# thnak/image_super_resolution

Hardware: AMD Instinct MI355X
Metric: 4x SR megapixels/sec (HR output) + PSNR vs reference CPU path (higher is better)
Workload: dtype fp16; 1 GPU; ResNet(16, 0.2, scaleRate=4) RRDB inference, 128x128->512x512; global_batch=16, per_gpu_batch=16, lr_size=128, scale=4, parallelism=dp1 (independent tile shards), streams_per_gpu=1, hip_graph=True, trunk=persistent chain kernel, storage=fp16 activations and packed weights, fp32 accumulation

## Files before the change

### image_super_resolution_amd/csrc/trunk.hip

```cpp
#include "trunk_common.h"

namespace isr {

size_t trunk_state_words(int n, int ha, int wa) {
    const size_t tiles = (size_t)n * (ha / tk::TH) * (wa / tk::TW);
    return trunk_rec_off((int)tiles) + 1024 * 16;
}

__global__ __launch_bounds__(1024) void trunk_prep_kernel(const isr_conv_desc* layers, const int32_t* kinds, int nl,
                                                          int n, int ha, int wa, unsigned* state, int th,
                                                          int h16) {
    extern __shared__ __attribute__((aligned(16))) char smem[];
    unsigned* err = reinterpret_cast<unsigned*>(smem);
    const int L = threadIdx.x;
    const int nbx = wa / tk::TW, nby = ha / th, ntiles = n * nbx * nby;
    const size_t ro = trunk_rec_off(ntiles);
    if (L == 0) *err = 0;
    __syncthreads();
    const isr_conv_desc& g0 = layers[0];
    if (L < nl) {
        const isr_conv_desc& d = layers[L];
        unsigned e = 0;
        auto same_geo = [&](const isr_view& v) {
            return v.hp == g0.x.hp && v.wp == g0.x.wp && v.cs == g0.x.cs && v.pad == g0.x.pad && v.coff % 16 == 0 &&
                   v.pad >= 1;
        };
        const int kind = kinds[L];
        const bool masked = kind == 2;
        if (d.n != n || d.ha != ha || d.wa != wa || d.h != g0.h || d.w != g0.w) e |= 1;
        if (!same_geo(d.x) || !same_geo(d.y) || (d.r2.data && !same_geo(d.r2)) || (masked && !same_geo(d.m))) e |= 2;
        if (kind == 0 || kind == 2 ? d.cout != 32 : (kind == 1 ? d.cout != 64 : true)) e |= 4;
        if (d.cin % 16 || d.cin < 64 || d.cin / 16 > 120 || !d.bias || ((uintptr_t)d.bias & 15)) e |= 8;
        if (d.f16 != h16 || d.shuffle != 1 || d.x_sub2 || d.taps || d.y2.data || (d.m.data != nullptr) != masked ||
            (masked && (d.m_c0 != 0 || d.slope != 1.f || d.r1.data || d.r2.data || d.s1 != 1.f || d.s2 != 1.f)))
            e |= 16;
        int fold = 0;
        uint16_t idv = 0;
        if (d.r1.data) {
            const float inv = 1.f / d.s1;
            float back;
            if (h16) {
                const _Float16 hi = (_Float16)inv;
                idv = __builtin_bit_cast(uint16_t, hi);
                back = (float)hi;
            } else {
                const __bf16 bi = (__bf16)inv;
                idv = __builtin_bit_cast(uint16_t, bi);
                back = (float)bi;
            }
            const bool alias = d.r1.data == d.x.data && d.r1.coff == d.x.coff && d.r1_cn == 0;
            if (!alias || kind != 1 || d.slope != 1.f || back != inv) e |= 32;
            fold = 1;
        } else if (d.r2.data) {
            e |= 32;
        }
        int first_new = tk::NEED_NONE;
        if (L > 0) {
            const isr_conv_desc& p = layers[L - 1];
            const int lo = p.y.coff, hi = p.y.coff + p.cout;
            first_new = d.cin / 16;
            if (p.y.data == d.x.data) {
                for (int c = 0; c < d.cin / 16; ++c) {
                    const int c0 = d.x.coff + 16 * c;
                    if (c0 < hi && lo < c0 + 16) {
                        first_new = c;
                        break;
                    }
                }
            }
        }
        TrunkRec rec;
        rec.x = (uint64_t)(uintptr_t)d.x.data;
        rec.y = (uint64_t)(uintptr_t)d.y.data;
        rec.w = (uint64_t)(uintptr_t)d.wpack;
        rec.b = (uint64_t)(uintptr_t)d.bias;
        rec.r2 = (uint64_t)(uintptr_t)(masked ? d.m.data : d.r2.data);
        rec.planes = (uint32_t)(d.x.coff / 16) | (uint32_t)(d.y.coff / 16) << 16;
        rec.shape = (uint32_t)((masked ? d.m.coff : d.r2.coff) / 16) | (uint32_t)(d.cin / 16) << 16 |
                    (uint32_t)(kind & 255) << 24;
        int form = EPI_GENERAL;
        if (kind == 0 && !d.r1.data && !d.r2.data && d.s2 == 1.f && d.slope > 0.f && d.slope < 1.f)
            form = EPI_GROWTH;
        else if (kind == 1 && fold && d.slope == 1.f)
            form = d.r2.data ? EPI_FINAL_R2 : (d.s2 == 1.f ? EPI_FINAL : EPI_FINAL_S2);
        rec.deps = (uint32_t)first_new | (uint32_t)fold << 8 | (uint32_t)form << 9 | (uint32_t)idv << 16;
        rec.slope = masked ? d.mslope : d.slope;
        rec.s1 = d.s1;
        rec.s2 = d.s2;
        const uint32_t* src = reinterpret_cast<const uint32_t*>(&rec);
        uint32_t* dst = state + ro + (size_t)L * 16;
#pragma unroll
        for (int i = 0; i < 16; ++i) dst[i] = src[i];
        if (e) atomicOr(err, e);
    }
    __syncthreads();
    if (L == 0) {
        const size_t plane = (size_t)g0.x.hp * g0.x.wp * 32;
        const unsigned e = *err | (plane >= 0x7fffffffull ? 64u : 0u) | (nl > 1024 ? 128u : 0u);
        uint32_t* geo = state + ro - 16;
        const int32_t gv[16] = {n, g0.h, g0.w, ha, wa, g0.x.hp, g0.x.wp, g0.x.cs / 16, g0.x.pad, nbx, nby, ntiles,
                                (int32_t)e, 0, 0, 0};
#pragma unroll
        for (int i = 0; i < 16; ++i) geo[i] = (uint32_t)gv[i];
        state[0] = state[0] + 1u;
    }
}

int trunk_prep_launch(const isr_chain_desc* cd, int th, hipStream_t s) {
    hipLaunchKernelGGL(trunk_prep_kernel, dim3(1), dim3(1024), 16, s, cd->layers, cd->kinds, cd->nl, cd->n, cd->ha,
                       cd->wa, cd->state, th, cd->f16 ? 1 : 0);
    return hipGetLastError() == hipSuccess ? 0 : -1;
}

#ifdef ISR_TUNING
__device__ unsigned long long* g_trunk_stamps;
#endif
__device__ __forceinline__ void trunk_stamp(int L, int t, int ntiles, int slot) {
#ifdef ISR_TUNING
    unsigned long long* p = g_trunk_stamps;
    if (p != nullptr && threadIdx.x == 0 && L >= 75 && L < 90) {
        unsigned long long v;
        asm volatile("s_memrealtime %0\n\ts_waitcnt lgkmcnt(0)" : "=s"(v)::"memory");
        p[((size_t)(L - 75) * ntiles + t) * 8 + slot] = v;
    }
#else
    (void)L, (void)t, (void)ntiles, (void)slot;
#endif
}

#ifdef ISR_TUNING
__device__ int g_trunk_knobs[4];
static int g_trunk_per_cu = 0;
__device__ __forceinline__ int trunk_abl_load() { return __builtin_amdgcn_readfirstlane(g_trunk_knobs[0]); }
#else
__device__ __forceinline__ int trunk_abl_load() { return 0; }
#endif

#ifdef ISR_TUNING
__device__ unsigned long long* g_item_stamps;
#endif
__device__ __forceinline__ void item_stamp(int L, int first_tile, int ch, int slot, int wm) {
#ifdef ISR_TUNING
    unsigned long long* p = g_item_stamps;
    const int w = wave_id();
    if (p != nullptr && first_tile && (threadIdx.x & 63) == 0 && (w == 0 || w == wm / 2) && (L == 77 || L == 79)) {
        const unsigned long long v = __builtin_amdgcn_s_memtime();
        p[((((size_t)blockIdx.x * 2 + (L == 79)) * 16 + ch) * 2 + (w != 0)) * 8 + slot] = v;
    }
#else
    (void)L, (void)first_tile, (void)ch, (void)slot, (void)wm;
#endif
}

struct TrunkArgs {
    unsigned* state;
    int rec_off;
    int nl;
    int acquire;
};


__device__ __forceinline__ void glds4(const void* gsrc, void* lds) {
    __builtin_amdgcn_global_load_lds(gsrc, ISR_LDS_PTR(lds), 4, 0, 0);
}

struct TK {
    static constexpr int WM = 4, R = 4, NST = 2;
    static constexpr int HALO_AUX = 16, STORE_AUX = 16;
    static constexpr int NT = 64 * WM;
    static constexpr int TH = tk::TH;
    static constexpr int HQ = (TH + 2) * tk::HC;
    static constexpr int HP = (HQ + 31) / 32;
    static_assert(R * WM == TH, "the waves cover the tile rows");
    static constexpr int HPW = (HP + WM - 1) / WM;
    static constexpr int WPW = (tk::WPF + WM - 1) / WM;
    static constexpr int SLOT = (HP + tk::WPF) * 1024;
    static constexpr int BIAS_OFF = NST * SLOT;
    static constexpr int LDS = BIAS_OFF + 4 * 256;
    static constexpr int BPC = 2;
    static_assert(BPC * LDS <= 163840, "LDS budget");
    static constexpr int WPS = BPC * WM / 4;
};

struct Src {
    const char* x;
    uint32_t h0;
    const char* w;
    const float* b;
    int wpc;
    uint32_t xbytes, wbytes;
};

struct TrunkCtx {
    unsigned* state;
    unsigned gen;
    int acquire;
    int hp, wp, cs16, pad, h, w, nbx, nby, ntiles;
    uint32_t pstride;
    uint32_t hoff[TK::HPW];
    int abl;
};

__device__ __forceinline__ Src src_of(const TrunkCtx& c, const_rec& rec, int t) {
    const int bx = t % c.nbx, tmp = t / c.nbx, by = tmp % c.nby, img = tmp / c.nby;
    Src s;
    s.x = (const char*)(uintptr_t)rec.x + (size_t)((uint32_t)img * c.cs16 + rec_xp(rec)) * c.pstride;
    s.h0 = (uint32_t)(((by * TK::TH - 1 + c.pad) * c.wp + (bx * tk::TW - 1 + c.pad)) * 32);
    s.w = (const char*)(uintptr_t)rec.w;
    s.b = (const float*)(uintptr_t)rec.b;
    s.wpc = rec_kind(rec) == 1 ? tk::WPF : tk::WPG;
    s.xbytes = c.pstride;
    s.wbytes = (uint32_t)(rec_nch(rec) * s.wpc * 1024);
    return s;
}

__device__ __forceinline__ uint32_t stage_pieces(const uint32_t* hoff, uint32_t pstride, int abl, const Src& s,
                                                 int chunk, int slot, bool with_bias, int bslot) {
    extern __shared__ __attribute__((aligned(16))) char smem[];
    const int wave = wave_id(), lane = threadIdx.x & 63;
    char* dst = smem + slot * TK::SLOT;
    uint32_t n = 0;
    const auto rx = rsrc_n(s.x + (size_t)chunk * pstride, s.xbytes);
    const uint32_t so = s.h0;
    if (!(abl & 1)) {
#pragma unroll
        for (int k = 0; k < TK::HPW; ++k) {
            const int j = wave + TK::WM * k;
            if (j < TK::HP) {
                __builtin_amdgcn_raw_ptr_buffer_load_lds(rx, ISR_LDS_PTR(dst + j * 1024), 16, hoff[k], so, 0, TK::HALO_AUX);
                ++n;
            }
        }
    }
    const auto rw = rsrc_n(s.w, s.wbytes);
    const uint32_t wo = (uint32_t)(chunk * s.wpc * 1024);
    char* wd = dst + TK::HP * 1024;
#pragma unroll
    for (int k = 0; k < TK::WPW; ++k) {
        const int j = wave + TK::WM * k;
        if (j < s.wpc && !(abl & 8)) {
            __builtin_amdgcn_raw_ptr_buffer_load_lds(rw, ISR_LDS_PTR(wd + j * 1024), 16, lane * 16, wo + j * 1024, 0, 0);
            ++n;
        }
    }
    if (with_bias && wave == 0) {
        if (lane < (s.wpc == tk::WPG ? 32 : 64))
            __builtin_amdgcn_raw_ptr_buffer_load_lds(rsrc_n(s.b, s.wpc == tk::WPG ? 128u : 256u),
                                                     ISR_LDS_PTR(smem + TK::BIAS_OFF + bslot * 256), 4, lane * 4, 0, 0, 0);
        ++n;
    }
    return n;
}

__device__ __forceinline__ uint32_t stage_chunk(const TrunkCtx& c, const Src& s, int chunk, int slot, bool with_bias,
                                                int bslot) {
#ifdef ISR_TUNING
    if (chunk < 0 || (uint32_t)(chunk * s.wpc * 1024) >= s.wbytes || slot < 0 || slot >= TK::NST ||
        bslot < 0 || bslot > 3) {
        if (threadIdx.x == 0) {
            __hip_atomic_store(c.state + 1, c.gen, __ATOMIC_RELAXED, __HIP_MEMORY_SCOPE_AGENT);
            __hip_atomic_fetch_add(c.state + 2, 1u, __ATOMIC_RELAXED, __HIP_MEMORY_SCOPE_AGENT);
        }
        return 0;
    }
#endif
    return stage_pieces(c.hoff, c.pstride, c.abl, s, chunk, slot, with_bias, bslot);
}

struct Next {
    bool exists;
    int L, t;
    Src src;
    int first_new;
    int nch;
    bool self_dep;
};

struct Stream {
    int item;
    int staged;
    int tseq;
    uint32_t issued;
    uint32_t m0, m1, m2, m3;
    int pend_t;
    unsigned pend_v;
    uint32_t pend_mark;
    bool dep_next;
};

__device__ __forceinline__ void push_mark(Stream& st) {
    const int pos = st.staged - st.item;
    const uint32_t v = st.issued;
    st.m0 = pos == 0 ? v : st.m0;
    st.m1 = pos == 1 ? v : st.m1;
    st.m2 = pos == 2 ? v : st.m2;
    st.m3 = pos >= 3 ? v : st.m3;
}

__device__ __forceinline__ void pop_mark(Stream& st) {
    st.m0 = st.m1;
    st.m1 = st.m2;
    st.m2 = st.m3;
}

__device__ __forceinline__ void force_publish(const TrunkCtx& c, Stream& st) {
    if (st.pend_t < 0) return;
    asm volatile("s_waitcnt vmcnt(0)" ::: "memory");
    raw_barrier();
    if (threadIdx.x == 0)
        __hip_atomic_store(c.state + 4 + st.pend_t, st.pend_v, __ATOMIC_RELAXED, __HIP_MEMORY_SCOPE_AGENT);
    st.pend_t = -1;
}

__device__ __forceinline__ bool next_item(int L, int t, int b, int G, int ntiles, int nl, int& nL, int& nt) {
    nL = L;
    nt = t;
    if (t + G < ntiles) {
        nt = t + G;
        return true;
    }
    if (L + 1 < nl) {
        nL = L + 1;
        nt = b;
        return true;
    }
    return false;
}

__device__ __forceinline__ bool tiles_adjacent(const TrunkCtx& c, int t, int t2) {
    const int bx = t % c.nbx, tq = t / c.nbx, by = tq % c.nby, im = tq / c.nby;
    const int bx2 = t2 % c.nbx, nq = t2 / c.nbx, by2 = nq % c.nby, im2 = nq / c.nby;
    return im == im2 && abs(bx - bx2) <= 1 && abs(by - by2) <= 1;
}

enum : int {
    CR_GENERAL,
    CR_FIRST,
    CR_SECOND,
    CR_STEADY,
    CR_DEP,
    CR_LOOP,
    CR_LAST
};

template <int NF, bool MASKED = false, bool H = false>
__device__ __forceinline__ void run_tile(const TrunkCtx& c, Stream& st, const_rec* recs, int L, int t,
                                         int nxL, int nxt, bool nx_exists) {
    extern __shared__ __attribute__((aligned(16))) char smem[];
    constexpr int R = TK::R, NST = TK::NST, CT = 32 * NF, TN = 3, NA = R + 2;
    constexpr bool ROLES = !MASKED;
    constexpr bool FULL = ROLES && NF == 1;
    constexpr int WPC = NF == 2 ? tk::WPF : tk::WPG;
    const_rec& rec = recs[L];
    const int wave = wave_id(), lane = threadIdx.x & 63, l31 = lane & 31, hh = lane >> 5;
    const int bx = t % c.nbx, tmp = t / c.nbx, by = tmp % c.nby, img = tmp / c.nby;
    const int x0 = bx * tk::TW, y0 = by * TK::TH;
    const int nch = rec_nch(rec);
    const int first_new = rec_first_new(rec);
    const unsigned need = c.gen * 1024u + (unsigned)L;
    const bool fold = NF == 2 && rec_fold(rec);
    const bool has_r2 = NF == 2 && rec.r2 != 0;
    constexpr bool masked = NF == 1 && MASKED;
    const Src me = src_of(c, rec, t);
    Next nx;
    if constexpr (!ROLES) {
        const_rec& nrec = recs[nxL];
        nx.exists = nx_exists;
        nx.L = nxL;
        nx.t = nxt;
        nx.src = src_of(c, nrec, nxt);
        nx.first_new = rec_first_new(nrec);
        nx.nch = rec_nch(nrec);
        nx.self_dep = tiles_adjacent(c, t, nxt);
    }
    const char* xn = me.x;
    uint32_t wo = 0;
    bool dep_ok = first_new == tk::NEED_NONE || st.dep_next;
    st.dep_next = false;
    const int bslot = st.tseq & 3;
    const int first_item = st.item;
    trunk_stamp(L, t, c.ntiles, 0);

    const uint32_t a_w = (uint32_t)(TK::HP * 1024 + (2 * l31 + (hh ^ ((l31 >> 3) & 1))) * 16);
    uint32_t a_h[3];
#pragma unroll
    for (int dx = 0; dx < 3; ++dx)
        a_h[dx] = (uint32_t)((wave * R * tk::HC + l31 + dx) * 32 + 16 * (hh ^ (((l31 + dx) >> 3) & 1)));

    auto wait_deps = [&](int tt, unsigned nd) {
        force_publish(c, st);
        trunk_stamp(L, t, c.ntiles, 4);
        if (!(c.abl & 16)) dep_wait(c.state, nb_of(tt, c.nbx, c.nby), nd, c.gen);
        if (c.acquire) acquire_fence();
        trunk_stamp(L, t, c.ntiles, 5);
    };

    auto stage_own = [&](const int sl) {
        char* dst = smem + sl * TK::SLOT;
        uint32_t n = 0;
        const auto rx = rsrc_n(xn, c.pstride);
        if (!(c.abl & 1)) {
#pragma unroll
            for (int k = 0; k < TK::HPW; ++k) {
                const int j = wave + TK::WM * k;
                if (TK::WM * k + TK::WM <= TK::HP || j < TK::HP) {
                    __builtin_amdgcn_raw_ptr_buffer_load_lds(rx, ISR_LDS_PTR(dst + j * 1024), 16, c.hoff[k], me.h0, 0,
                                                             TK::HALO_AUX);
                    ++n;
                }
            }
        }
        if (!(c.abl & 8)) {
            const auto rw = rsrc_n(me.w, me.wbytes);
#pragma unroll
            for (int k = 0; k < (WPC + TK::WM - 1) / TK::WM; ++k) {
                const int j = wave + TK::WM * k;
                if (TK::WM * k + TK::WM <= WPC || j < WPC) {
                    __builtin_amdgcn_raw_ptr_buffer_load_lds(rw, ISR_LDS_PTR(dst + (TK::HP + j) * 1024), 16, lane * 16,
                                                             wo + j * 1024, 0, 0);
                    ++n;
                }
            }
        }
        xn += c.pstride;
        wo += WPC * 1024;
        return n;
    };

    f32x16 acc[R][NF];

    const uint32_t idv = rec_idv(rec);
    auto do_chunk = [&](const int ch, auto fc_tag, auto s_tag, auto role_tag) {
        constexpr int FC = decltype(fc_tag)::value, S = decltype(s_tag)::value, ROLE = decltype(role_tag)::value;
        static_assert((ROLE == CR_GENERAL) == MASKED, "the masked layers run the general chunk");
            const int slot = S >= 0 ? S : st.item % NST;
            const bool stamp_tile = t == (int)blockIdx.x;
            item_stamp(L, stamp_tile, ch, 0, TK::WM);
            bool ring_ok = true;
            if constexpr (ROLE == CR_FIRST) {
                if (st.staged < st.item) {
                    force_publish(c, st);
                    if (first_new == 0 && !dep_ok) {
                        wait_deps(t, need);
                        dep_ok = true;
                    }
                    st.issued += stage_chunk(c, me, 0, slot, true, bslot);
                    st.staged = st.item;
                    st.m0 = st.issued;
                }
                xn += c.pstride;
                wo += WPC * 1024;
                wait_vm_coarse(st.issued - st.m0);
            } else if constexpr (ROLE != CR_GENERAL) {
#ifdef ISR_TUNING
                if (st.issued != st.m0) {
                    ring_ok = false;
                    if (threadIdx.x == 0) {
                        __hip_atomic_store(c.state + 1, c.gen, __ATOMIC_RELAXED, __HIP_MEMORY_SCOPE_AGENT);
                        __hip_atomic_fetch_add(c.state + 2, 1u, __ATOMIC_RELAXED, __HIP_MEMORY_SCOPE_AGENT);
                    }
                }
#endif
                asm volatile("s_waitcnt vmcnt(0)" ::: "memory");
            } else {
            if (st.staged < st.item) {
                force_publish(c, st);
                if (ch >= first_new && !dep_ok) {
                    wait_deps(t, need);
                    dep_ok = true;
                }
                st.issued += stage_chunk(c, me, ch, slot, ch == 0, bslot);
                st.staged = st.item;
                push_mark(st);
            }
            wait_vm(st.issued - st.m0);
            }
            item_stamp(L, stamp_tile, ch, 1, TK::WM);
            raw_barrier();
            item_stamp(L, stamp_tile, ch, 2, TK::WM);
            if constexpr (ROLE == CR_GENERAL || ROLE == CR_FIRST || ROLE == CR_SECOND) {
            if (st.pend_t >= 0 && (int)(st.m0 - st.pend_mark) >= 0) {
                if (threadIdx.x == 0)
                    __hip_atomic_store(c.state + 4 + st.pend_t, st.pend_v, __ATOMIC_RELAXED, __HIP_MEMORY_SCOPE_AGENT);
                st.pend_t = -1;
            }
            }
            if (ROLE == CR_FIRST || (ROLE == CR_GENERAL && ch == 0)) {
                trunk_stamp(L, t, c.ntiles, 1);
                const float* bs = reinterpret_cast<const float*>(smem + TK::BIAS_OFF + bslot * 256);
    #pragma unroll
                for (int f = 0; f < NF; ++f) {
                    f32x16 b0;
    #pragma unroll
                    for (int j = 0; j < 4; ++j) {
                        const f32x4 q = *reinterpret_cast<const f32x4*>(bs + f * 32 + 8 * j + 4 * hh);
    #pragma unroll
                        for (int e = 0; e < 4; ++e) b0[4 * j + e] = q[e];
                    }
    #pragma unroll
                    for (int r = 0; r < R; ++r) acc[r][f] = b0;
                }
            }
            const char* sb = smem + slot * TK::SLOT;
            bf16x8 fb[2][TN][NF], fa[2][NA];
            auto read_one = [&](int dx, int idx, int set) {
                if (idx < TN * NF) {
                    const int dyi = idx / NF, f = idx % NF;
                    fb[set][dyi][f] = lds_read16(sb + a_w + ((dyi * 3 + dx) * CT * 2 + f * 64) * 16);
                } else {
                    const int ia = idx - TN * NF;
                    fa[set][ia] = lds_read16(sb + a_h[dx] + ia * tk::HC * 32);
                }
            };
            auto read_fb = [&](int dx, int dyi, int set) {
    #pragma unroll
                for (int f = 0; f < NF; ++f) read_one(dx, dyi * NF + f, set);
            };
            auto read_step0 = [&]() {
                read_fb(0, 0, 0);
    #pragma unroll
                for (int ia = 0; ia < R; ++ia) read_one(0, TN * NF + ia, 0);
                read_fb(0, 1, 0);
                read_one(0, TN * NF + R, 0);
                read_fb(0, 2, 0);
                read_one(0, TN * NF + R + 1, 0);
                __builtin_amdgcn_sched_barrier(0);
            };
            read_step0();

            const bool last = ROLE == CR_LAST || (ROLE == CR_LOOP && ch == nch - 1);
            if constexpr (ROLE == CR_LAST || ROLE == CR_LOOP) {
                if (last && nx_exists && ring_ok) {
                    const_rec& nrec = recs[nxL];
                    bool go = true;
                    if (nxL > 0 && rec_first_new(nrec) == 0) {
                        if (tiles_adjacent(c, t, nxt)) {
                            go = false;
                        } else {
                            wait_deps(nxt, c.gen * 1024u + (unsigned)nxL);
                            st.dep_next = true;
                        }
                    }
                    if (go) {
                        st.issued += stage_chunk(c, src_of(c, nrec, nxt), 0, slot ^ 1, true, (bslot + 1) & 3);
                        ++st.staged;
                        st.m1 = st.issued;
                    }
                }
            }
            if constexpr (ROLE != CR_GENERAL && ROLE != CR_LAST) {
                if constexpr (ROLE != CR_STEADY) {
                    if (!last && ch + 1 >= first_new && !dep_ok) {
                        wait_deps(t, need);
                        dep_ok = true;
                    }
                }
                if (!last && ring_ok) {
                    st.issued += stage_own(slot ^ 1);
                    ++st.staged;
                    st.m1 = st.issued;
                }
            }
            if constexpr (ROLE == CR_GENERAL)
            while (st.staged < st.item + NST - 1) {
                const int off = st.staged + 1 - first_item;
                const int nslot = (st.staged + 1) % NST;
                if (off < nch) {
                    if (off >= first_new && !dep_ok) {
                        wait_deps(t, need);
                        dep_ok = true;
                    }
                    st.issued += stage_chunk(c, me, off, nslot, false, 0);
                } else {
                    const int nc = off - nch;
                    if (!nx.exists || nc >= nx.nch) break;
                    if (nx.L > 0 && nc >= nx.first_new && !st.dep_next) {
                        if (nx.self_dep) break;
                        wait_deps(nx.t, c.gen * 1024u + (unsigned)nx.L);
                        st.dep_next = true;
                    }
                    st.issued += stage_chunk(c, nx.src, nc, nslot, nc == 0, (bslot + 1) & 3);
                }
                ++st.staged;
                push_mark(st);
            }
            __builtin_amdgcn_sched_barrier(0);
            item_stamp(L, stamp_tile, ch, 3, TK::WM);
            __builtin_amdgcn_s_setprio(1);

    #pragma unroll
            for (int stp = 0; stp < 3; ++stp) {
                const int cur = stp & 1;
    #pragma unroll
                for (int dyi = 0; dyi < TN; ++dyi) {
    #pragma unroll
                    for (int r = 0; r < R; ++r) {
    #pragma unroll
                        for (int f = 0; f < NF; ++f) acc[r][f] = mfma32t<H>(fb[cur][dyi][f], fa[cur][r + dyi], acc[r][f]);
                        if constexpr (NF == 2 && FC >= 0) {
                            if (dyi == 1 && stp == 1) {
                                const bf16x8 a = fold_a_bits(idv, FC & 1);
                                acc[r][FC >> 1] = mfma32t<H>(a, fa[cur][r + 1], acc[r][FC >> 1]);
                            }
                        }
                        if (stp + 1 < 3 && (dyi == 2 || r == 0)) read_one(stp + 1, TN * NF + r + dyi, cur ^ 1);
                        __builtin_amdgcn_sched_barrier(0);
                    }
                    if (stp + 1 < 3) {
                        read_fb(stp + 1, dyi, cur ^ 1);
                        __builtin_amdgcn_sched_barrier(0);
                    }
                }
            }
            __builtin_amdgcn_s_setprio(0);
            item_stamp(L, stamp_tile, ch, 4, TK::WM);
            pop_mark(st);
            ++st.item;
    };
    if constexpr (ROLES) {
        int ch = 0;
        auto in_slot = [&](auto fc_tag, auto role_tag) {
            if constexpr (!FULL) do_chunk(ch, fc_tag, TIC<-1>{}, role_tag);
            else if (st.item & 1) do_chunk(ch, fc_tag, TIC<1>{}, role_tag);
            else do_chunk(ch, fc_tag, TIC<0>{}, role_tag);
            ++ch;
        };
        if constexpr (NF == 2) {
            if (fold) {
                in_slot(TIC<0>{}, TIC<CR_FIRST>{});
                in_slot(TIC<1>{}, TIC<CR_SECOND>{});
                in_slot(TIC<2>{}, TIC<CR_DEP>{});
                in_slot(TIC<3>{}, TIC<CR_LOOP>{});
            }
        }
        if (ch == 0) {
            in_slot(TIC<-1>{}, TIC<CR_FIRST>{});
            in_slot(TIC<-1>{}, TIC<CR_SECOND>{});
        }
        if (ch < nch) {
            const int wb = first_new - 1;
            int stop = wb >= ch && wb < nch - 1 ? wb : nch - 1;
            if constexpr (!FULL) {
                for (; ch < nch; ++ch) do_chunk(ch, TIC<-1>{}, TIC<-1>{}, TIC<CR_LOOP>{});
            } else {
                for (;;) {
                    if (ch < stop && (st.item & 1)) {
                        do_chunk(ch, TIC<-1>{}, TIC<1>{}, TIC<CR_STEADY>{});
                        ++ch;
                    }
                    for (; ch + 1 < stop; ch += 2) {
                        do_chunk(ch, TIC<-1>{}, TIC<0>{}, TIC<CR_STEADY>{});
                        do_chunk(ch + 1, TIC<-1>{}, TIC<1>{}, TIC<CR_STEADY>{});
                    }
                    if (ch < stop) {
                        do_chunk(ch, TIC<-1>{}, TIC<0>{}, TIC<CR_STEADY>{});
                        ++ch;
                    }
                    if (ch >= nch - 1) break;
                    in_slot(TIC<-1>{}, TIC<CR_DEP>{});
                    stop = nch - 1;
                }
                in_slot(TIC<-1>{}, TIC<CR_LAST>{});
            }
        }
    } else {
        for (int ch = 0; ch < nch; ++ch) do_chunk(ch, TIC<-1>{}, TIC<-1>{}, TIC<CR_GENERAL>{});
    }
    trunk_stamp(L, t, c.ntiles, 2);

    if (!dep_ok && first_new != tk::NEED_NONE) wait_deps(t, need);

    auto epilogue = [&](auto form_tag, auto full_tag) {
        constexpr int EF = decltype(form_tag)::value;
        constexpr bool GEN = EF == EPI_GENERAL, FT = decltype(full_tag)::value != 0;
        static_assert(GEN || (EF == EPI_GROWTH ? NF == 1 && !MASKED : NF == 2), "form and layer kind");
        const bool use_r2 = GEN ? (has_r2 || masked) : EF == EPI_FINAL_R2;
        float zero = 0.f;
        if constexpr (EF == EPI_GROWTH) asm volatile("; trunk epilogue form %1 full %2" : "+s"(zero) : "n"(EF), "n"((int)FT));
        else if constexpr (!GEN) asm volatile("; trunk epilogue form %0 full %1" ::"n"(EF), "n"((int)FT));
        typedef __attribute__((ext_vector_type(4))) unsigned u32x4;
        const int xx = x0 + l31;
        const float slope = rec.slope, s1 = rec.s1, s2 = rec.s2;
        const bool scale2 = s2 != 1.f;
        const char* ybase = (const char*)(uintptr_t)rec.y + (size_t)((uint32_t)img * c.cs16 + rec_yp(rec)) * c.pstride;
        bf16x8 q2[R][NF][2];
        const char* r2base = (const char*)(uintptr_t)rec.r2 + (size_t)((uint32_t)img * c.cs16 + rec_r2p(rec)) * c.pstride;
        auto load_r2 = [&](int r) {
            const uint32_t pix = (uint32_t)((y0 + wave * R + r + c.pad) * c.wp + xx + c.pad);
#pragma unroll
            for (int f = 0; f < NF; ++f)
#pragma unroll
                for (int blk = 0; blk < 2; ++blk) {
                    const auto rr = rsrc_n(r2base + (size_t)(2 * f + blk) * c.pstride, c.pstride);
                    q2[r][f][blk] = __builtin_bit_cast(
                        bf16x8, __builtin_amdgcn_raw_buffer_load_b128(rr, pix * 32 + 16 * hh, 0, 16));
                }
            st.issued += NF * 2;
        };
        if (use_r2) load_r2(0);
#pragma unroll
        for (int r = 0; r < R; ++r) {
            if (use_r2 && r + 1 < R) load_r2(r + 1);
            const int yy = y0 + wave * R + r;
            const bool valid = yy < c.h && xx < c.w;
            const uint32_t pix = (uint32_t)((yy + c.pad) * c.wp + xx + c.pad);
#pragma unroll
            for (int f = 0; f < NF; ++f) {
                float v[16];
                if constexpr (GEN) {
#pragma unroll
                    for (int g = 0; g < 16; ++g) v[g] = acc[r][f][g];
                } else {
                    typedef __attribute__((ext_vector_type(2))) float f32x2;
                    const f32x16& a = acc[r][f];
#pragma unroll
                    for (int g = 0; g < 16; g += 2) {
                        f32x2 p = {a[g], a[g + 1]};
                        if constexpr (EF == EPI_GROWTH) {
                            p = p * slope;
                        } else {
                            p = p * s1;
                            if constexpr (EF == EPI_FINAL_S2) p = p * s2;
                        }
                        v[g] = p[0];
                        v[g + 1] = p[1];
                    }
                    if constexpr (EF == EPI_GROWTH) {
#pragma unroll
                        for (int g = 0; g < 16; ++g) v[g] = a[g] >= zero ? a[g] : v[g];
                    }
                }
#pragma unroll
                for (int k = 0; k < 4; ++k) {
                    swap_halves(v[k], v[4 + k]);
                    swap_halves(v[8 + k], v[12 + k]);
                }
#pragma unroll
                for (int blk = 0; blk < 2; ++blk) {
                    float* u = v + 8 * blk;
#pragma unroll
                    for (int e = 0; e < 8; ++e) {
                        if constexpr (!GEN) {
                            if constexpr (EF == EPI_FINAL_R2) u[e] = __builtin_fmaf(u[e], s2, elt<H>(q2[r][f][blk], e));
                        } else {
                        if (masked)
                            u[e] = elt<H>(q2[r][f][blk], e) > 0.f ? u[e] : u[e] * slope;
                        else
                            u[e] = u[e] >= 0.f ? u[e] : u[e] * slope;
                        if (fold) u[e] = u[e] * s1;
                        if (has_r2) {
                            u[e] = u[e] * s2 + elt<H>(q2[r][f][blk], e);
                        } else {
                            if (scale2) u[e] *= s2;
                        }
                        if (!valid) u[e] = 0.f;
                        }
                    }
                    const auto yr = rsrc_n(ybase + (size_t)(2 * f + blk) * c.pstride, c.pstride);
                    const uint32_t off = pix * 32 + 16 * hh;
                    bf16x8 tq;
                    if constexpr (GEN) {
                        tq = pack8<H>(u);
                    } else {
                        tq = pack8_pairs<H>(u);
                        if constexpr (!FT) {
                            u32x4 z = __builtin_bit_cast(u32x4, tq);
#pragma unroll
                            for (int d = 0; d < 4; ++d) z[d] = valid ? z[d] : 0u;
                            tq = __builtin_bit_cast(bf16x8, z);
                        }
                    }
                    if (!(c.abl & 4)) {
                        __builtin_amdgcn_raw_buffer_store_b128(__builtin_bit_cast(u32x4, tq), yr, off, 0, TK::STORE_AUX);
                        ++st.issued;
                    }
                }
            }
        }
    };
    auto epilogue_of = [&](auto form_tag) {
        if (y0 + TK::TH <= c.h && x0 + tk::TW <= c.w) epilogue(form_tag, TIC<1>{});
        else epilogue(form_tag, TIC<0>{});
    };
    const int form = ROLES ? rec_form(rec) : (int)EPI_GENERAL;
    if constexpr (ROLES && NF == 1) {
        if (form == EPI_GROWTH) epilogue_of(TIC<EPI_GROWTH>{});
        else epilogue(TIC<EPI_GENERAL>{}, TIC<0>{});
    } else if constexpr (ROLES) {
        if (form == EPI_FINAL) epilogue_of(TIC<EPI_FINAL>{});
        else if (form == EPI_FINAL_R2) epilogue_of(TIC<EPI_FINAL_R2>{});
        else if (form == EPI_FINAL_S2) epilogue_of(TIC<EPI_FINAL_S2>{});
        else epilogue(TIC<EPI_GENERAL>{}, TIC<0>{});
    } else {
        epilogue(TIC<EPI_GENERAL>{}, TIC<0>{});
    }
    trunk_stamp(L, t, c.ntiles, 3);
    st.pend_t = t;
    st.pend_v = c.gen * 1024u + (unsigned)(L + 1);
    st.pend_mark = st.issued;
    ++st.tseq;
}

template <bool H>
__global__ __launch_bounds__(TK::NT, TK::WPS) void trunk_kernel(TrunkArgs a) {
    TrunkCtx c;
    c.state = a.state;
    c.acquire = a.acquire;
    c.gen = __hip_atomic_load(a.state, __ATOMIC_RELAXED, __HIP_MEMORY_SCOPE_AGENT);
    const_geo& g = *(const_geo*)(uintptr_t)(a.state + a.rec_off - 16);
    const_rec* recs = (const_rec*)(uintptr_t)(a.state + a.rec_off);
    if (g.err != 0) {
        if (threadIdx.x == 0) {
            __hip_atomic_store(a.state + 1, c.gen, __ATOMIC_RELAXED, __HIP_MEMORY_SCOPE_AGENT);
            __hip_atomic_fetch_add(a.state + 2, 1u, __ATOMIC_RELAXED, __HIP_MEMORY_SCOPE_AGENT);
        }
        return;
    }
    c.hp = g.hp;
    c.wp = g.wp;
    c.cs16 = g.cs16;
    c.pad = g.pad;
    c.h = g.h;
    c.w = g.w;
    c.nbx = g.nbx;
    c.nby = g.nby;
    c.ntiles = g.ntiles;
    c.pstride = (uint32_t)(c.hp * c.wp * 32);
    c.abl = trunk_abl_load();
    {
        const int wave = wave_id(), lane = threadIdx.x & 63;
#pragma unroll
        for (int k = 0; k < TK::HPW; ++k) c.hoff[k] = halo_piece_off<TK::HQ>(wave + TK::WM * k, lane, c.wp);
    }
    const int G = gridDim.x, b = (int)blockIdx.x;
    Stream st;
    st.item = 0;
    st.staged = 0;
    st.tseq = 0;
    st.issued = 0;
    st.m0 = st.m1 = st.m2 = st.m3 = 0;
    st.pend_t = -1;
    st.pend_v = 0;
    st.pend_mark = 0;
    st.dep_next = false;
    if (b < c.ntiles) {
        st.issued += stage_chunk(c, src_of(c, recs[0], b), 0, 0, true, 0);
        st.m0 = st.issued;
        for (int L = 0; L < a.nl; ++L) {
            const_rec& rec = recs[L];
            for (int t = b; t < c.ntiles; t += G) {
                int nxL, nxt;
                const bool nx_exists = next_item(L, t, b, G, c.ntiles, a.nl, nxL, nxt);
                const int kind = rec_kind(rec);
                if (kind == 0) run_tile<1, false, H>(c, st, recs, L, t, nxL, nxt, nx_exists);
                else if (kind == 2) run_tile<1, true, H>(c, st, recs, L, t, nxL, nxt, nx_exists);
                else run_tile<2, false, H>(c, st, recs, L, t, nxL, nxt, nx_exists);
            }
        }
    }
    asm volatile("s_waitcnt vmcnt(0)" ::: "memory");
    __syncthreads();
    if (threadIdx.x == 0 && st.pend_t >= 0)
        __hip_atomic_store(c.state + 4 + st.pend_t, st.pend_v, __ATOMIC_RELAXED, __HIP_MEMORY_SCOPE_AGENT);
}

template <bool H>
static int trunk_launch_k(const isr_chain_desc* cd, hipStream_t s) {
    if (cd->ha % TK::TH || cd->wa % tk::TW || cd->nl < 1 || cd->nl > 1024) return -2;
    const int nbx = cd->wa / tk::TW, nby = cd->ha / TK::TH;
    const long long ntiles = (long long)cd->n * nbx * nby;
    if (ntiles <= 0 || ntiles > (1 << 24)) return -2;
    static thread_local int cached_dev = -1, cached_per_cu = 0, cached_cus = 0;
    int dev = 0;
    if (hipGetDevice(&dev) != hipSuccess) return -1;
    const void* kern = (const void*)trunk_kernel<H>;
    if (dev != cached_dev) {
        (void)hipFuncSetAttribute(kern, hipFuncAttributeMaxDynamicSharedMemorySize, TK::LDS);
        int per_cu = 0;
        if (hipOccupancyMaxActiveBlocksPerMultiprocessor(&per_cu, kern, TK::NT, TK::LDS) != hipSuccess) return -1;
        int cus = 0;
        if (hipDeviceGetAttribute(&cus, hipDeviceAttributeMultiprocessorCount, dev) != hipSuccess || cus <= 0) return -1;
        cached_dev = dev;
        cached_per_cu = per_cu < TK::BPC ? per_cu : TK::BPC;
        cached_cus = cus;
    }
    int per_cu = cached_per_cu;
#ifdef ISR_TUNING
    if (g_trunk_per_cu > 0 && g_trunk_per_cu < per_cu) per_cu = g_trunk_per_cu;
#endif
    if (per_cu < 1) return -4;
    const long long slots = (long long)per_cu * cached_cus;
    const int grid = (int)(ntiles < slots ? ntiles : slots);
    const int rec_off = (int)trunk_rec_off((int)ntiles);
    trunk_prep_launch(cd, TK::TH, s);
    TrunkArgs a;
    a.state = cd->state;
    a.rec_off = rec_off;
    a.nl = cd->nl;
    a.acquire = cd->acquire;
    hipLaunchKernelGGL((trunk_kernel<H>), dim3(grid), dim3(TK::NT), TK::LDS, s, a);
    return hipGetLastError() == hipSuccess ? 0 : -1;
}

int trunk_launch(const isr_chain_desc* cd, hipStream_t s) {
    return cd->f16 ? trunk_launch_k<true>(cd, s) : trunk_launch_k<false>(cd, s);
}

#ifdef ISR_TUNING
int trunk_knobs_set(const int* k) {
    g_trunk_per_cu = k[1];
    return hipMemcpyToSymbol(HIP_SYMBOL(g_trunk_knobs), k, 4 * sizeof(int)) == hipSuccess ? 0 : -1;
}
int trunk_stamps_set(void* p) { return hipMemcpyToSymbol(HIP_SYMBOL(g_trunk_stamps), &p, sizeof(p)) == hipSuccess ? 0 : -1; }
int trunk_item_stamps_set(void* p) {
    return hipMemcpyToSymbol(HIP_SYMBOL(g_item_stamps), &p, sizeof(p)) == hipSuccess ? 0 : -1;
}
#else
int trunk_knobs_set(const int*) { return -2; }
int trunk_stamps_set(void*) { return -2; }
int trunk_item_stamps_set(void*) { return -2; }
#endif

}
```

### image_super_resolution_amd/csrc/trunk_common.h

```cpp
#pragma once
#include "isr_common.h"

namespace isr {

namespace tk {
constexpr int TH = 16;
constexpr int TW = 32;
constexpr int HR = TH + 2, HC = TW + 2, HQ = HR * HC;
constexpr int HP = (HQ + 31) / 32;
constexpr int WPG = 9, WPF = 18;
constexpr int NEED_NONE = 255;
}

struct TrunkRec {
    uint64_t x, y, w, b, r2;
    uint32_t planes;
    uint32_t shape;
    uint32_t deps;
    float slope, s1, s2;
};
static_assert(sizeof(TrunkRec) == 64, "record size");

enum : int {
    EPI_GENERAL,
    EPI_GROWTH,
    EPI_FINAL,
    EPI_FINAL_S2,
    EPI_FINAL_R2
};

struct TrunkGeo {
    int32_t n, h, w, ha, wa, hp, wp, cs16, pad, nbx, nby, ntiles, err, r0, r1, r2;
};

static inline __host__ __device__ size_t trunk_rec_off(int ntiles) {
    return ((size_t)ntiles + 4 + 15) / 16 * 16 + 16;
}

size_t trunk_state_words(int n, int ha, int wa);

typedef const __attribute__((address_space(4))) TrunkRec const_rec;
typedef const __attribute__((address_space(4))) TrunkRec const_rec_t;
typedef const __attribute__((address_space(4))) TrunkGeo const_geo;
__device__ __forceinline__ int rec_xp(const_rec_t& r) { return (int)(r.planes & 0xffff); }
__device__ __forceinline__ int rec_yp(const_rec_t& r) { return (int)(r.planes >> 16); }
__device__ __forceinline__ int rec_r2p(const_rec_t& r) { return (int)(r.shape & 0xffff); }
__device__ __forceinline__ int rec_nch(const_rec_t& r) { return (int)((r.shape >> 16) & 255); }
__device__ __forceinline__ int rec_kind(const_rec_t& r) { return (int)(r.shape >> 24); }
__device__ __forceinline__ int rec_first_new(const_rec_t& r) { return (int)(r.deps & 255); }
__device__ __forceinline__ bool rec_fold(const_rec_t& r) { return ((r.deps >> 8) & 1) != 0; }
__device__ __forceinline__ int rec_form(const_rec_t& r) { return (int)((r.deps >> 9) & 7); }
__device__ __forceinline__ uint32_t rec_idv(const_rec_t& r) { return r.deps >> 16; }

__device__ __forceinline__ void raw_barrier() {
    asm volatile("s_waitcnt lgkmcnt(0)" ::: "memory");
    __builtin_amdgcn_s_barrier();
}

__device__ __forceinline__ int nb_of(int t, int nbx, int nby) {
    const int lane = threadIdx.x & 63;
    if (lane >= 9) return -1;
    const int bx = t % nbx, tmp = t / nbx, by = tmp % nby, img = tmp / nby;
    const int yy = by + lane / 3 - 1, xx = bx + lane % 3 - 1;
    return (yy >= 0 && yy < nby && xx >= 0 && xx < nbx) ? (img * nby + yy) * nbx + xx : -1;
}

constexpr int kTrunkSpinSleep = 1;

__device__ __forceinline__ unsigned poll_load(const unsigned* progress, int nb) {
    return __hip_atomic_load(progress + (nb < 0 ? 0 : nb), __ATOMIC_RELAXED, __HIP_MEMORY_SCOPE_AGENT);
}

__device__ __forceinline__ void dep_wait(unsigned* state, int nb, unsigned need, unsigned gen) {
    const unsigned* progress = state + 4;
    for (unsigned spins = 0;; ++spins) {
        const unsigned v = poll_load(progress, nb);
        if (__all(nb < 0 || (int)(v - need) >= 0)) break;
        if ((spins & 255) == 255 && __hip_atomic_load(state + 1, __ATOMIC_RELAXED, __HIP_MEMORY_SCOPE_AGENT) == gen)
            break;
        if (spins > (1u << 18)) {
            if ((threadIdx.x & 63) == 0) {
                __hip_atomic_store(state + 1, gen, __ATOMIC_RELAXED, __HIP_MEMORY_SCOPE_AGENT);
                __hip_atomic_fetch_add(state + 2, 1u, __ATOMIC_RELAXED, __HIP_MEMORY_SCOPE_AGENT);
            }
            break;
        }
        __builtin_amdgcn_s_sleep(kTrunkSpinSleep);
    }
}

__device__ __forceinline__ void acquire_fence() {
    if ((threadIdx.x & 63) == 0) __builtin_amdgcn_fence(__ATOMIC_ACQUIRE, "agent");
    asm volatile("s_waitcnt vmcnt(0)" ::: "memory");
}

__device__ __forceinline__ __amdgpu_buffer_rsrc_t rsrc_n(const void* p, uint32_t bytes) {
    return __builtin_amdgcn_make_buffer_rsrc(const_cast<void*>(p), (short)0, (int)bytes, 0x00020000);
}

template <int HQ>
__device__ __forceinline__ uint32_t halo_piece_off(int j, int lane, int wp) {
    const int u = j * 64 + lane;
    const int q = u >> 1;
    if (q >= HQ) return 0;
    const int row = q / tk::HC, col = q - row * tk::HC;
    const int cc = (u & 1) ^ ((col >> 3) & 1);
    return (uint32_t)((row * wp + col) * 32 + cc * 16);
}

__device__ __forceinline__ void wait_vm(uint32_t n) {
#define ISR_VMW(k)                                        \
    case k:                                               \
        asm volatile("s_waitcnt vmcnt(" #k ")" ::: "memory"); \
        break;
    switch (n) {
        ISR_VMW(1) ISR_VMW(2) ISR_VMW(3) ISR_VMW(4) ISR_VMW(5) ISR_VMW(6) ISR_VMW(7) ISR_VMW(8) ISR_VMW(9)
        ISR_VMW(10) ISR_VMW(11) ISR_VMW(12) ISR_VMW(13) ISR_VMW(14) ISR_VMW(15) ISR_VMW(16) ISR_VMW(17)
        ISR_VMW(18) ISR_VMW(19) ISR_VMW(20) ISR_VMW(21) ISR_VMW(22) ISR_VMW(23) ISR_VMW(24) ISR_VMW(25)
        ISR_VMW(26) ISR_VMW(27) ISR_VMW(28) ISR_VMW(29) ISR_VMW(30) ISR_VMW(31) ISR_VMW(32) ISR_VMW(33)
        ISR_VMW(34) ISR_VMW(35) ISR_VMW(36) ISR_VMW(37) ISR_VMW(38) ISR_VMW(39) ISR_VMW(40) ISR_VMW(41)
        ISR_VMW(42) ISR_VMW(43) ISR_VMW(44) ISR_VMW(45) ISR_VMW(46) ISR_VMW(47) ISR_VMW(48) ISR_VMW(49)
        ISR_VMW(50) ISR_VMW(51) ISR_VMW(52) ISR_VMW(53) ISR_VMW(54) ISR_VMW(55) ISR_VMW(56) ISR_VMW(57)
        ISR_VMW(58) ISR_VMW(59) ISR_VMW(60) ISR_VMW(61) ISR_VMW(62) ISR_VMW(63)
        default: asm volatile("s_waitcnt vmcnt(0)" ::: "memory"); break;
    }
#undef ISR_VMW
}

__device__ __forceinline__ void wait_vm_coarse(uint32_t n) {
    if (n >= 16) asm volatile("s_waitcnt vmcnt(16)" ::: "memory");
    else if (n >= 8) asm volatile("s_waitcnt vmcnt(8)" ::: "memory");
    else asm volatile("s_waitcnt vmcnt(0)" ::: "memory");
}

template <int V> struct TIC { static constexpr int value = V; };

__device__ __forceinline__ bf16x8 fold_a_bits(uint32_t idv, int h16) {
    const int lane = threadIdx.x & 63;
    const int j = (lane & 31) - 16 * h16 - 8 * (lane >> 5);
    typedef __attribute__((ext_vector_type(4))) unsigned u32x4;
    u32x4 r;
#pragma unroll
    for (int d = 0; d < 4; ++d) r[d] = j == 2 * d ? idv : (j == 2 * d + 1 ? idv << 16 : 0u);
    return __builtin_bit_cast(bf16x8, r);
}

int trunk_prep_launch(const isr_chain_desc* cd, int th, hipStream_t s);

}
```

Before: 669.3 MPix/s.

## Pair consecutive dense-block growth convolutions into one fused 64-channel pass

Adds a pairing mode to the persistent trunk chain. Two consecutive growth convs that read the same input planes are run together. The first phase computes both layers' 32 output channels over the shared input channels, with alternate waves staging each layer's weights. The second phase finishes only the extra 32 channels of the second layer, starting from the carried accumulators. This cuts halo loads and dependency waits for the shared input chunks and halves the per-tile passes over the common prefix. In exchange it adds register pressure from carried accumulators, more complex staging and dependency logic, and a heuristic gate based on grid size.

```diff
diff --git a/image_super_resolution_amd/csrc/trunk.hip b/image_super_resolution_amd/csrc/trunk.hip
--- a/image_super_resolution_amd/csrc/trunk.hip
+++ b/image_super_resolution_amd/csrc/trunk.hip
@@ -9,13 +9,20 @@
 
 __global__ __launch_bounds__(1024) void trunk_prep_kernel(const isr_conv_desc* layers, const int32_t* kinds, int nl,
                                                           int n, int ha, int wa, unsigned* state, int th,
-                                                          int h16) {
+                                                          int h16, int grid, int pair_mode) {
     extern __shared__ __attribute__((aligned(16))) char smem[];
+    __shared__ unsigned char pairable[1024];
+    __shared__ unsigned npaired;
     unsigned* err = reinterpret_cast<unsigned*>(smem);
     const int L = threadIdx.x;
     const int nbx = wa / tk::TW, nby = ha / th, ntiles = n * nbx * nby;
     const size_t ro = trunk_rec_off(ntiles);
-    if (L == 0) *err = 0;
+    const bool pairs_ok = pair_mode != TRUNK_PAIRS_OFF && pairs_allowed(ntiles, nbx, nby, n, grid);
+    if (L == 0) {
+        *err = 0;
+        npaired = 0;
+    }
+    pairable[L] = 0;
     __syncthreads();
     const isr_conv_desc& g0 = layers[0];
     if (L < nl) {
@@ -92,6 +99,28 @@
 #pragma unroll
         for (int i = 0; i < 16; ++i) dst[i] = src[i];
         if (e) atomicOr(err, e);
+        if (pairs_ok && !e && form == EPI_GROWTH && L + 1 < nl && kinds[L + 1] == 0) {
+            const isr_conv_desc& q = layers[L + 1];
+            const bool q_growth = !q.r1.data && !q.r2.data && q.s2 == 1.f && q.slope > 0.f && q.slope < 1.f;
+            const bool shared = q.x.data == d.x.data && q.x.coff == d.x.coff && q.cin == d.cin + 32;
+            const bool feeds = d.y.data == d.x.data && d.y.coff == d.x.coff + d.cin;
+            const bool wanted = pair_mode >= TRUNK_PAIRS_ALL || d.cin / 16 >= 8;
+            pairable[L] = q_growth && shared && feeds && wanted && q.cout == 32 && q.f16 == h16;
+        }
+    }
+    __syncthreads();
+    if (L < nl) {
+        auto first_of_pair = [&](int i) {
+            if (i < 0 || !pairable[i]) return false;
+            int s = i;
+            while (s > 0 && pairable[s - 1]) --s;
+            return ((i - s) & 1) == 0;
+        };
+        const unsigned pb = first_of_pair(L) ? 1u : (first_of_pair(L - 1) ? 2u : 0u);
+        if (pb) {
+            state[ro + (size_t)L * 16 + 12] |= pb << 12;
+            atomicAdd(&npaired, 1u);
+        }
     }
     __syncthreads();
     if (L == 0) {
@@ -99,16 +128,16 @@
         const unsigned e = *err | (plane >= 0x7fffffffull ? 64u : 0u) | (nl > 1024 ? 128u : 0u);
         uint32_t* geo = state + ro - 16;
         const int32_t gv[16] = {n, g0.h, g0.w, ha, wa, g0.x.hp, g0.x.wp, g0.x.cs / 16, g0.x.pad, nbx, nby, ntiles,
-                                (int32_t)e, 0, 0, 0};
+                                (int32_t)e, (int32_t)npaired, 0, 0};
 #pragma unroll
         for (int i = 0; i < 16; ++i) geo[i] = (uint32_t)gv[i];
         state[0] = state[0] + 1u;
     }
 }
 
-int trunk_prep_launch(const isr_chain_desc* cd, int th, hipStream_t s) {
+int trunk_prep_launch(const isr_chain_desc* cd, int th, int grid, int pair_mode, hipStream_t s) {
     hipLaunchKernelGGL(trunk_prep_kernel, dim3(1), dim3(1024), 16, s, cd->layers, cd->kinds, cd->nl, cd->n, cd->ha,
-                       cd->wa, cd->state, th, cd->f16 ? 1 : 0);
+                       cd->wa, cd->state, th, cd->f16 ? 1 : 0, grid, pair_mode);
     return hipGetLastError() == hipSuccess ? 0 : -1;
 }
 
@@ -189,6 +218,7 @@
     const float* b;
     int wpc;
     uint32_t xbytes, wbytes;
+    const_rec* pb;
 };
 
 struct TrunkCtx {
@@ -211,6 +241,11 @@
     s.wpc = rec_kind(rec) == 1 ? tk::WPF : tk::WPG;
     s.xbytes = c.pstride;
     s.wbytes = (uint32_t)(rec_nch(rec) * s.wpc * 1024);
+    s.pb = nullptr;
+    if (rec_pair(rec) == 1) {
+        s.pb = &rec + 1;
+        s.wpc = tk::WPF;
+    }
     return s;
 }
 
@@ -232,21 +267,38 @@
             }
         }
     }
-    const auto rw = rsrc_n(s.w, s.wbytes);
-    const uint32_t wo = (uint32_t)(chunk * s.wpc * 1024);
+    static_assert(TK::WM % 2 == 0, "pair staging: a wave's pieces all come from one pack");
+    const bool pair = s.pb != nullptr, second = pair && (wave & 1);
+    const char* wsrc = s.w;
+    uint32_t wext = s.wbytes;
+    if (second) {
+        wsrc = (const char*)(uintptr_t)s.pb->w;
+        wext += 2 * tk::WPG * 1024;
+    }
+    const auto rw = rsrc_n(wsrc, wext);
+    const uint32_t wo = (uint32_t)(chunk * (pair ? tk::WPG : s.wpc) * 1024);
     char* wd = dst + TK::HP * 1024;
 #pragma unroll
     for (int k = 0; k < TK::WPW; ++k) {
         const int j = wave + TK::WM * k;
         if (j < s.wpc && !(abl & 8)) {
-            __builtin_amdgcn_raw_ptr_buffer_load_lds(rw, ISR_LDS_PTR(wd + j * 1024), 16, lane * 16, wo + j * 1024, 0, 0);
+            __builtin_amdgcn_raw_ptr_buffer_load_lds(rw, ISR_LDS_PTR(wd + j * 1024), 16, lane * 16,
+                                                     wo + (pair ? j >> 1 : j) * 1024, 0, 0);
             ++n;
         }
     }
     if (with_bias && wave == 0) {
-        if (lane < (s.wpc == tk::WPG ? 32 : 64))
-            __builtin_amdgcn_raw_ptr_buffer_load_lds(rsrc_n(s.b, s.wpc == tk::WPG ? 128u : 256u),
-                                                     ISR_LDS_PTR(smem + TK::BIAS_OFF + bslot * 256), 4, lane * 4, 0, 0, 0);
+        char* bd = smem + TK::BIAS_OFF + bslot * 256;
+        if (pair) {
+            if (lane < 32) {
+                __builtin_amdgcn_raw_ptr_buffer_load_lds(rsrc_n(s.b, 128u), ISR_LDS_PTR(bd), 4, lane * 4, 0, 0, 0);
+                __builtin_amdgcn_raw_ptr_buffer_load_lds(rsrc_n((const float*)(uintptr_t)s.pb->b, 128u), ISR_LDS_PTR(bd + 128), 4, lane * 4, 0, 0, 0);
+            }
+            ++n;
+        } else if (lane < (s.wpc == tk::WPG ? 32 : 64)) {
+            __builtin_amdgcn_raw_ptr_buffer_load_lds(rsrc_n(s.b, s.wpc == tk::WPG ? 128u : 256u), ISR_LDS_PTR(bd), 4,
+                                                     lane * 4, 0, 0, 0);
+        }
         ++n;
     }
     return n;
@@ -255,7 +307,7 @@
 __device__ __forceinline__ uint32_t stage_chunk(const TrunkCtx& c, const Src& s, int chunk, int slot, bool with_bias,
                                                 int bslot) {
 #ifdef ISR_TUNING
-    if (chunk < 0 || (uint32_t)(chunk * s.wpc * 1024) >= s.wbytes || slot < 0 || slot >= TK::NST ||
+    if (chunk < 0 || (uint32_t)(chunk * (s.pb ? tk::WPG : s.wpc) * 1024) >= s.wbytes || slot < 0 || slot >= TK::NST ||
         bslot < 0 || bslot > 3) {
         if (threadIdx.x == 0) {
             __hip_atomic_store(c.state + 1, c.gen, __ATOMIC_RELAXED, __HIP_MEMORY_SCOPE_AGENT);
@@ -312,15 +364,15 @@
     st.pend_t = -1;
 }
 
-__device__ __forceinline__ bool next_item(int L, int t, int b, int G, int ntiles, int nl, int& nL, int& nt) {
+__device__ __forceinline__ bool next_item(int L, int step, int t, int b, int G, int ntiles, int nl, int& nL, int& nt) {
     nL = L;
     nt = t;
     if (t + G < ntiles) {
         nt = t + G;
         return true;
     }
-    if (L + 1 < nl) {
-        nL = L + 1;
+    if (L + step < nl) {
+        nL = L + step;
         nt = b;
         return true;
     }
@@ -343,14 +395,16 @@
     CR_LAST
 };
 
-template <int NF, bool MASKED = false, bool H = false>
+template <int NF, bool MASKED = false, bool H = false, int PH = 0>
 __device__ __forceinline__ void run_tile(const TrunkCtx& c, Stream& st, const_rec* recs, int L, int t,
-                                         int nxL, int nxt, bool nx_exists) {
+                                         int nxL, int nxt, bool nx_exists, f32x16* pacc = nullptr) {
     extern __shared__ __attribute__((aligned(16))) char smem[];
     constexpr int R = TK::R, NST = TK::NST, CT = 32 * NF, TN = 3, NA = R + 2;
     constexpr bool ROLES = !MASKED;
+    static_assert(PH == 0 || (!MASKED && NF == (PH == 1 ? 2 : 1)), "pair phases: 64-cout bodies, then 32-cout");
     constexpr bool FULL = ROLES && NF == 1;
     constexpr int WPC = NF == 2 ? tk::WPF : tk::WPG;
+    constexpr int WSTEP = PH == 1 ? tk::WPG : WPC;
     const_rec& rec = recs[L];
     const int wave = wave_id(), lane = threadIdx.x & 63, l31 = lane & 31, hh = lane >> 5;
     const int bx = t % c.nbx, tmp = t / c.nbx, by = tmp % c.nby, img = tmp / c.nby;
@@ -358,8 +412,8 @@
     const int nch = rec_nch(rec);
     const int first_new = rec_first_new(rec);
     const unsigned need = c.gen * 1024u + (unsigned)L;
-    const bool fold = NF == 2 && rec_fold(rec);
-    const bool has_r2 = NF == 2 && rec.r2 != 0;
+    const bool fold = NF == 2 && PH == 0 && rec_fold(rec);
+    const bool has_r2 = NF == 2 && PH == 0 && rec.r2 != 0;
     constexpr bool masked = NF == 1 && MASKED;
     const Src me = src_of(c, rec, t);
     Next nx;
@@ -373,9 +427,18 @@
         nx.nch = rec_nch(nrec);
         nx.self_dep = tiles_adjacent(c, t, nxt);
     }
-    const char* xn = me.x;
-    uint32_t wo = 0;
-    bool dep_ok = first_new == tk::NEED_NONE || st.dep_next;
+    const int ch0 = PH == 2 ? nch - 2 : 0;
+    const char* w_own = me.w;
+    uint32_t wext_own = me.wbytes;
+    if constexpr (PH == 1) {
+        if (wave & 1) {
+            w_own = (const char*)(uintptr_t)recs[L + 1].w;
+            wext_own += 2 * tk::WPG * 1024;
+        }
+    }
+    const char* xn = me.x + (size_t)ch0 * c.pstride;
+    uint32_t wo = (uint32_t)(ch0 * WSTEP * 1024);
+    bool dep_ok = PH != 2 && (first_new == tk::NEED_NONE || st.dep_next);
     st.dep_next = false;
     const int bslot = st.tseq & 3;
     const int first_item = st.item;
@@ -411,23 +474,27 @@
             }
         }
         if (!(c.abl & 8)) {
-            const auto rw = rsrc_n(me.w, me.wbytes);
+            const auto rw = rsrc_n(w_own, wext_own);
 #pragma unroll
             for (int k = 0; k < (WPC + TK::WM - 1) / TK::WM; ++k) {
                 const int j = wave + TK::WM * k;
                 if (TK::WM * k + TK::WM <= WPC || j < WPC) {
                     __builtin_amdgcn_raw_ptr_buffer_load_lds(rw, ISR_LDS_PTR(dst + (TK::HP + j) * 1024), 16, lane * 16,
-                                                             wo + j * 1024, 0, 0);
+                                                             wo + (PH == 1 ? j >> 1 : j) * 1024, 0, 0);
                     ++n;
                 }
             }
         }
         xn += c.pstride;
-        wo += WPC * 1024;
+        wo += WSTEP * 1024;
         return n;
     };
 
     f32x16 acc[R][NF];
+    if constexpr (PH == 2) {
+#pragma unroll
+        for (int r = 0; r < R; ++r) acc[r][0] = pacc[r];
+    }
 
     const uint32_t idv = rec_idv(rec);
     auto do_chunk = [&](const int ch, auto fc_tag, auto s_tag, auto role_tag) {
@@ -440,16 +507,16 @@
             if constexpr (ROLE == CR_FIRST) {
                 if (st.staged < st.item) {
                     force_publish(c, st);
-                    if (first_new == 0 && !dep_ok) {
+                    if ((PH == 2 || first_new == 0) && !dep_ok) {
                         wait_deps(t, need);
                         dep_ok = true;
                     }
-                    st.issued += stage_chunk(c, me, 0, slot, true, bslot);
+                    st.issued += stage_chunk(c, me, ch, slot, PH != 2, bslot);
                     st.staged = st.item;
                     st.m0 = st.issued;
                 }
                 xn += c.pstride;
-                wo += WPC * 1024;
+                wo += WSTEP * 1024;
                 wait_vm_coarse(st.issued - st.m0);
             } else if constexpr (ROLE != CR_GENERAL) {
 #ifdef ISR_TUNING
@@ -485,7 +552,7 @@
                 st.pend_t = -1;
             }
             }
-            if (ROLE == CR_FIRST || (ROLE == CR_GENERAL && ch == 0)) {
+            if (PH != 2 && (ROLE == CR_FIRST || (ROLE == CR_GENERAL && ch == 0))) {
                 trunk_stamp(L, t, c.ntiles, 1);
                 const float* bs = reinterpret_cast<const float*>(smem + TK::BIAS_OFF + bslot * 256);
     #pragma unroll
@@ -529,7 +596,7 @@
             read_step0();
 
             const bool last = ROLE == CR_LAST || (ROLE == CR_LOOP && ch == nch - 1);
-            if constexpr (ROLE == CR_LAST || ROLE == CR_LOOP) {
+            if constexpr ((ROLE == CR_LAST || ROLE == CR_LOOP) && PH != 1) {
                 if (last && nx_exists && ring_ok) {
                     const_rec& nrec = recs[nxL];
                     bool go = true;
@@ -618,14 +685,18 @@
             ++st.item;
     };
     if constexpr (ROLES) {
-        int ch = 0;
+        int ch = ch0;
         auto in_slot = [&](auto fc_tag, auto role_tag) {
             if constexpr (!FULL) do_chunk(ch, fc_tag, TIC<-1>{}, role_tag);
             else if (st.item & 1) do_chunk(ch, fc_tag, TIC<1>{}, role_tag);
             else do_chunk(ch, fc_tag, TIC<0>{}, role_tag);
             ++ch;
         };
-        if constexpr (NF == 2) {
+        if constexpr (PH == 2) {
+            in_slot(TIC<-1>{}, TIC<CR_FIRST>{});
+            in_slot(TIC<-1>{}, TIC<CR_LAST>{});
+        }
+        if constexpr (NF == 2 && PH == 0) {
             if (fold) {
                 in_slot(TIC<0>{}, TIC<CR_FIRST>{});
                 in_slot(TIC<1>{}, TIC<CR_SECOND>{});
@@ -633,10 +704,12 @@
                 in_slot(TIC<3>{}, TIC<CR_LOOP>{});
             }
         }
+        if constexpr (PH != 2)
         if (ch == 0) {
             in_slot(TIC<-1>{}, TIC<CR_FIRST>{});
             in_slot(TIC<-1>{}, TIC<CR_SECOND>{});
         }
+        if constexpr (PH != 2)
         if (ch < nch) {
             const int wb = first_new - 1;
             int stop = wb >= ch && wb < nch - 1 ? wb : nch - 1;
@@ -673,7 +746,8 @@
     auto epilogue = [&](auto form_tag, auto full_tag) {
         constexpr int EF = decltype(form_tag)::value;
         constexpr bool GEN = EF == EPI_GENERAL, FT = decltype(full_tag)::value != 0;
-        static_assert(GEN || (EF == EPI_GROWTH ? NF == 1 && !MASKED : NF == 2), "form and layer kind");
+        static_assert(GEN || (EF == EPI_GROWTH ? (NF == 1 || PH == 1) && !MASKED : NF == 2 && PH == 0),
+                      "form and layer kind");
         const bool use_r2 = GEN ? (has_r2 || masked) : EF == EPI_FINAL_R2;
         float zero = 0.f;
         if constexpr (EF == EPI_GROWTH) asm volatile("; trunk epilogue form %1 full %2" : "+s"(zero) : "n"(EF), "n"((int)FT));
@@ -705,7 +779,7 @@
             const bool valid = yy < c.h && xx < c.w;
             const uint32_t pix = (uint32_t)((yy + c.pad) * c.wp + xx + c.pad);
 #pragma unroll
-            for (int f = 0; f < NF; ++f) {
+            for (int f = 0; f < (PH == 1 ? 1 : NF); ++f) {
                 float v[16];
                 if constexpr (GEN) {
 #pragma unroll
@@ -783,7 +857,9 @@
         else epilogue(form_tag, TIC<0>{});
     };
     const int form = ROLES ? rec_form(rec) : (int)EPI_GENERAL;
-    if constexpr (ROLES && NF == 1) {
+    if constexpr (PH != 0) {
+        epilogue_of(TIC<EPI_GROWTH>{});
+    } else if constexpr (ROLES && NF == 1) {
         if (form == EPI_GROWTH) epilogue_of(TIC<EPI_GROWTH>{});
         else epilogue(TIC<EPI_GENERAL>{}, TIC<0>{});
     } else if constexpr (ROLES) {
@@ -798,7 +874,12 @@
     st.pend_t = t;
     st.pend_v = c.gen * 1024u + (unsigned)(L + 1);
     st.pend_mark = st.issued;
-    ++st.tseq;
+    if constexpr (PH == 1) {
+#pragma unroll
+        for (int r = 0; r < R; ++r) pacc[r] = acc[r][1];
+    } else {
+        ++st.tseq;
+    }
 }
 
 template <bool H>
@@ -846,13 +927,19 @@
     if (b < c.ntiles) {
         st.issued += stage_chunk(c, src_of(c, recs[0], b), 0, 0, true, 0);
         st.m0 = st.issued;
-        for (int L = 0; L < a.nl; ++L) {
+        for (int L = 0, step; L < a.nl; L += step) {
             const_rec& rec = recs[L];
+            const bool pair = rec_pair(rec) == 1 && L + 1 < a.nl;
+            step = pair ? 2 : 1;
             for (int t = b; t < c.ntiles; t += G) {
                 int nxL, nxt;
-                const bool nx_exists = next_item(L, t, b, G, c.ntiles, a.nl, nxL, nxt);
+                const bool nx_exists = next_item(L, step, t, b, G, c.ntiles, a.nl, nxL, nxt);
                 const int kind = rec_kind(rec);
-                if (kind == 0) run_tile<1, false, H>(c, st, recs, L, t, nxL, nxt, nx_exists);
+                if (pair) {
+                    f32x16 pacc[TK::R];
+                    run_tile<2, false, H, 1>(c, st, recs, L, t, nxL, nxt, nx_exists, pacc);
+                    run_tile<1, false, H, 2>(c, st, recs, L + 1, t, nxL, nxt, nx_exists, pacc);
+                } else if (kind == 0) run_tile<1, false, H>(c, st, recs, L, t, nxL, nxt, nx_exists);
                 else if (kind == 2) run_tile<1, true, H>(c, st, recs, L, t, nxL, nxt, nx_exists);
                 else run_tile<2, false, H>(c, st, recs, L, t, nxL, nxt, nx_exists);
             }
@@ -892,7 +979,8 @@
     const long long slots = (long long)per_cu * cached_cus;
     const int grid = (int)(ntiles < slots ? ntiles : slots);
     const int rec_off = (int)trunk_rec_off((int)ntiles);
-    trunk_prep_launch(cd, TK::TH, s);
+    static const int pair_mode = getenv("ISR_TRUNK_PAIRS") ? atoi(getenv("ISR_TRUNK_PAIRS")) : TRUNK_PAIRS_ALL;
+    trunk_prep_launch(cd, TK::TH, grid, pair_mode < 0 ? 0 : (pair_mode > 2 ? 2 : pair_mode), s);
     TrunkArgs a;
     a.state = cd->state;
     a.rec_off = rec_off;
diff --git a/image_super_resolution_amd/csrc/trunk_common.h b/image_super_resolution_amd/csrc/trunk_common.h
--- a/image_super_resolution_amd/csrc/trunk_common.h
+++ b/image_super_resolution_amd/csrc/trunk_common.h
@@ -1,5 +1,6 @@
 #pragma once
 #include "isr_common.h"
+#include "trunk_pairs.h"
 
 namespace isr {
 
@@ -50,6 +51,7 @@
 __device__ __forceinline__ int rec_first_new(const_rec_t& r) { return (int)(r.deps & 255); }
 __device__ __forceinline__ bool rec_fold(const_rec_t& r) { return ((r.deps >> 8) & 1) != 0; }
 __device__ __forceinline__ int rec_form(const_rec_t& r) { return (int)((r.deps >> 9) & 7); }
+__device__ __forceinline__ int rec_pair(const_rec_t& r) { return (int)((r.deps >> 12) & 15); }
 __device__ __forceinline__ uint32_t rec_idv(const_rec_t& r) { return r.deps >> 16; }
 
 __device__ __forceinline__ void raw_barrier() {
@@ -145,6 +147,6 @@
     return __builtin_bit_cast(bf16x8, r);
 }
 
-int trunk_prep_launch(const isr_chain_desc* cd, int th, hipStream_t s);
+int trunk_prep_launch(const isr_chain_desc* cd, int th, int grid, int pair_mode, hipStream_t s);
 
 }
diff --git a/image_super_resolution_amd/csrc/trunk_pairs.h b/image_super_resolution_amd/csrc/trunk_pairs.h
--- /dev/null
+++ b/image_super_resolution_amd/csrc/trunk_pairs.h
@@ -0,0 +1,23 @@
+#pragma once
+
+namespace isr {
+
+#if defined(__HIP__) || defined(__CUDACC__)
+#define ISR_PAIRS_HD __host__ __device__
+#else
+#define ISR_PAIRS_HD
+#endif
+
+static inline ISR_PAIRS_HD bool pairs_allowed(long long ntiles, int nbx, int nby, int n, int G) {
+    if (ntiles <= 0 || nbx <= 0 || nby <= 0 || n <= 0 || G <= 0) return false;
+    if (ntiles <= G) return true;
+    return 2ll * (nbx + 2) <= G;
+}
+
+enum : int {
+    TRUNK_PAIRS_OFF = 0,
+    TRUNK_PAIRS_LONG = 1,
+    TRUNK_PAIRS_ALL = 2
+};
+
+}
```

Result: faster. 677.5 MPix/s, median of 6 (+1.2%).
